# amin-abouee/apex-solver

Measured on AMD Instinct MI355X. Metric: ms per LM iter (Jacobian+Schur+solve), lower is better.
Workload: dtype f64; 1 GPU; final-13682 synthetic (13682 cameras / 4456117 landmarks / 28966251 observations); optimization_type=selfcal, camera_dof=9, schur_variant=sparse, s_tile_rows=856, s_tiles=8071, s_tiles_touched=4284, etree_levels=41, border_cameras=0, schur_form=4, variant_asked=Sparse, reason=, variant_choice=direct, parallelism=landmark-shard x1

## Files before the change

apex-solver_amd/csrc/chol_kernels.hip:

```cpp
#include <hip/hip_runtime.h>
#include <stdint.h>

#include "chol_kernels.h"
#include "device_reduce.hpp"
#include <algorithm>

namespace apex {

typedef double double4_t __attribute__((ext_vector_type(4)));

constexpr int NB = kNB;
constexpr int BS = 16;
constexpr int NBK = NB / BS;
constexpr int BP = 18;
constexpr int BSZ = BS * BP;
constexpr int NLB = NBK * (NBK + 1) / 2;

__device__ __forceinline__ int bidx(int bi, int bj) { return bi * (bi + 1) / 2 + bj; }

__device__ __forceinline__ double readlane_f64(double v, int src) {
    const int lo = __builtin_amdgcn_readlane(__double2loint(v), src);
    const int hi = __builtin_amdgcn_readlane(__double2hiint(v), src);
    return __hiloint2double(hi, lo);
}
// ... 183 lines not shown
                    Xm = __builtin_amdgcn_mfma_f64_16x16x4f64(-la, xb, Xm, 0, 0, 0);
                }
            }
            double* D = sA + bidx(kb, kb) * BSZ;
            double* Xd = sD + kb * BSZ;
#pragma unroll
            for (int r = 0; r < 4; ++r) {
                const int c = lk + 4 * r;
                D[lr * BP + c] = lr >= c ? Ls[r] : 0.0;
                Xd[c * BP + lr] = Xs[r];
            }
            if (isbad) *bad = 1;
            POTRF_STAMP();
        } else if (helper) {
            if (kb >= 1) {
                const int ks = kb - 1;
                for (int i = kb + 1 + hid; i < NBK; i += NH) {
                    double* Cb = sA + bidx(i, kb) * BSZ;
                    double4_t acc = blk_load_cd(Cb, lr, lk);
                    acc = blk_mma_nt(sA + bidx(i, ks) * BSZ, sA + bidx(kb, ks) * BSZ, acc, lr, lk, -1.0);
                    blk_store_cd(Cb, acc, lr, lk, 1.0);
                }
                const int m = NBK - 1 - kb;
                const int n_upd = m * (m + 1) / 2;
                for (int t = hid; t < n_upd; t += NH) {
                    int ii = 0;
                    while ((ii + 1) * (ii + 2) / 2 <= t) ++ii;
                    const int jj = t - ii * (ii + 1) / 2;
                    const int i = kb + 1 + ii, j = kb + 1 + jj;
                    double* Cb = sA + bidx(i, j) * BSZ;
                    double4_t acc = blk_load_cd(Cb, lr, lk);
                    acc = blk_mma_nt(sA + bidx(i, ks) * BSZ, sA + bidx(j, ks) * BSZ, acc, lr, lk, -1.0);
                    blk_store_cd(Cb, acc, lr, lk, 1.0);
                }
                const int r = ks;
                int nt = 0;
                for (int j = hid; j < r; j += NH, ++nt) {
                    double4_t acc = (double4_t){0.0, 0.0, 0.0, 0.0};
                    for (int k = j; k < r; ++k) {
                        const double* Y = (k == j) ? (sD + j * BSZ) : (sA + bidx(k, j) * BSZ);
                        acc = blk_mma_nn(sA + bidx(r, k) * BSZ, Y, acc, lr, lk);
                    }
                    T[nt] = acc;
                }
            }
        }
        __syncthreads();
        POTRF_STAMP();
        if (helper && kb >= 1) {
            const int r = kb - 1;
            int nt = 0;
            for (int j = hid; j < r; j += NH, ++nt) blk_store_cd(sA + bidx(r, j) * BSZ, T[nt], lr, lk, -1.0);
        }
        {
            const int m = NBK - 1 - kb;
            if (w == 0) {
                if (m > 0) {
                    double* N = sA + bidx(kb + 1, kb) * BSZ;
                    double4_t Lt = (double4_t){0.0, 0.0, 0.0, 0.0};
                    Lt = blk_mma_nt(sD + kb * BSZ, N, Lt, lr, lk, 1.0);
                    Dm = blk_load_cd_sym(sA + bidx(kb + 1, kb + 1) * BSZ, lr, lk);
#pragma unroll
                    for (int r = 0; r < 4; ++r) N[lr * BP + lk + 4 * r] = Lt[r];
#pragma unroll
                    for (int r = 0; r < 4; ++r) Dm = __builtin_amdgcn_mfma_f64_16x16x4f64(-Lt[r], Lt[r], Dm, 0, 0, 0);
                }
            } else if (helper) {
                const int t0 = m > 0 ? 1 : 0;
                for (int t = t0 + hid; t < m + kb; t += NH) {
                    if (t < m) {
                        double* P = sA + bidx(kb + 1 + t, kb) * BSZ;
                        double4_t acc = (double4_t){0.0, 0.0, 0.0, 0.0};
                        acc = blk_mma_nt(P, sD + kb * BSZ, acc, lr, lk, 1.0);
                        blk_store_cd(P, acc, lr, lk, 1.0);
                    } else {
                        const int k = t - m;
                        double* Bk = sA + bidx(kb, k) * BSZ;
                        blk_to_tile<COH>(Bk, A, rA, kb, k, lane, 64);
                        double4_t acc = (double4_t){0.0, 0.0, 0.0, 0.0};
                        acc = blk_mma_nn(sD + kb * BSZ, Bk, acc, lr, lk);
                        blk_store_cd(Bk, acc, lr, lk, 1.0);
                    }
                }
                if (hid == NH - 1) blk_to_tile<COH>(sA + bidx(kb, kb) * BSZ, A, rA, kb, kb, lane, 64);
            }
        }
        if (w == 0 || helper) {
            __builtin_amdgcn_fence(__ATOMIC_RELEASE, "workgroup");
            if (lane == 0) __hip_atomic_fetch_add(sync_cnt, 1, __ATOMIC_RELAXED, __HIP_MEMORY_SCOPE_WORKGROUP);
        }
        if (helper) {
            const int target = (kb + 1) * (NH + 1);
            while (__hip_atomic_load(sync_cnt, __ATOMIC_RELAXED, __HIP_MEMORY_SCOPE_WORKGROUP) < target) __builtin_amdgcn_s_sleep(0);
            __builtin_amdgcn_fence(__ATOMIC_ACQUIRE, "workgroup");
        }
        POTRF_STAMP();
    }
    __syncthreads();
    {
        const int r = NBK - 1;
        double4_t T[(NBK - 1 + NW - 1) / NW];
        int nt = 0;
        for (int j = w; j < r; j += NW, ++nt) {
            double4_t acc = (double4_t){0.0, 0.0, 0.0, 0.0};
            for (int k = j; k < r; ++k) {
                const double* Y = (k == j) ? (sD + j * BSZ) : (sA + bidx(k, j) * BSZ);
                acc = blk_mma_nn(sA + bidx(r, k) * BSZ, Y, acc, lr, lk);
            }
            T[nt] = acc;
        }
        __syncthreads();
        nt = 0;
        for (int j = w; j < r; j += NW, ++nt) blk_store_cd(sA + bidx(r, j) * BSZ, T[nt], lr, lk, -1.0);
        __syncthreads();
    }
#pragma unroll
    for (int bi = 0; bi < NBK; ++bi) {
        const int per_row = 8 * (bi + 1), cnt = 16 * per_row;
        for (int idx = tid; idx < cnt; idx += NT) {
            const int rr = idx / per_row, c2 = idx - rr * per_row;
            const int bj = c2 >> 3;
            const double* src = ((bj == bi) ? (sD + bi * BSZ) : (sA + bidx(bi, bj) * BSZ)) + rr * BP + 2 * (c2 & 7);
            double2 v; v.x = src[0]; v.y = src[1];
            tile_st2<COH>(Linv, rL, (16 * bi + rr) * NB + 2 * c2, v);
        }
    }
    if (tid == 0 && *bad) atomicCAS(fail, 0, K + 1);
    POTRF_STAMP();
}

template <int NW>
__global__ __launch_bounds__(64 * NW) void k_potrf_inv_mf(const PotrfTask* __restrict__ tasks, int* __restrict__ fail,
                                                          int* __restrict__ arrived) {
    if (arrived != nullptr && threadIdx.x == 0) __hip_atomic_fetch_add(arrived, 1, __ATOMIC_RELAXED, __HIP_MEMORY_SCOPE_AGENT);
    POTRF_STAMP();
    __shared__ double sA[NLB * BSZ];
    __shared__ double sD[NBK * BSZ];
    __shared__ int bad, sync_cnt;
    const PotrfTask pt = tasks[blockIdx.x];
    potrf_tile_mf<NW, false>(pt.A, pt.Linv, pt.K, fail, sA, sD, &bad, &sync_cnt);
}
#undef POTRF_STAMP

constexpr int KC = 16;
constexpr int STRIP = 48;
constexpr int NSTRIP = NB / STRIP;
constexpr int kGemmSmallMax = 56;

typedef double __attribute__((address_space(1)))* GlobalF64;
typedef const double __attribute__((address_space(1)))* GlobalCF64;
typedef double f64x2_t __attribute__((ext_vector_type(2)));
typedef const f64x2_t __attribute__((address_space(1)))* GlobalCF64x2;

template <bool TRI>
__global__ __launch_bounds__(256, 3) void k_tile_gemm_nt(const GemmTask* __restrict__ tasks, int n_units, double alpha, double beta) {
    constexpr int P4 = KC + 2;
    constexpr int IMG = (NB + STRIP) * P4;
    __shared__ double sm[IMG];
    const int per_xcd = (n_units + 7) >> 3;
    const int unit = (blockIdx.x & 7) * per_xcd + (blockIdx.x >> 3);
    if ((int)(blockIdx.x >> 3) >= per_xcd || unit >= n_units) return;
    GemmTask tg = tasks[unit / NSTRIP];
    const bool first = (reinterpret_cast<uintptr_t>(tg.C) & 1) != 0;
    tg.C = reinterpret_cast<double*>(reinterpret_cast<uintptr_t>(tg.C) & ~uintptr_t(7));
    const int strip = unit % NSTRIP;
    const int tid = threadIdx.x, lane = tid & 63, w = __builtin_amdgcn_readfirstlane(tid >> 6);
    const int lr = lane & 15, lk = lane >> 4;
    GlobalCF64 Ag = (GlobalCF64)tg.A + (size_t)strip * STRIP * NB;
    GlobalCF64 Bg = (GlobalCF64)tg.B;
    constexpr int NACC = TRI ? 9 : 7;
    int cb[3];
    if (TRI) { cb[0] = 16 * (8 - w); cb[1] = 16 * (1 + w); cb[2] = w == 3 ? 0 : -16; }
    else { cb[0] = 32 * w; cb[1] = 32 * w + 16; cb[2] = 128; }
    const bool extra = TRI ? (w == 3) : (w < 3);
    double4_t acc[NACC];
#pragma unroll
    for (int j = 0; j < NACC; ++j) acc[j] = (double4_t){0.0, 0.0, 0.0, 0.0};
    constexpr int C2 = KC / 2, NR = (NB + STRIP) * C2 / 256, RPR = 256 / C2;
    static_assert((NB + STRIP) * C2 % 256 == 0 && 256 % C2 == 0 && NR == 6 && RPR == 32, "staging loop assumes whole rounds");
    const int r0 = tid / C2, c2 = tid % C2;
    const unsigned offB = r0 * NB + 2 * c2, offA = (r0 + 16) * NB + 2 * c2;
    GlobalCF64 p4 = r0 < 16 ? Bg + (size_t)(r0 + 128) * NB + 2 * c2 : Ag + (size_t)(r0 - 16) * NB + 2 * c2;
    const int dst0 = r0 * P4 + 2 * c2;
    f64x2_t rg[NR];
    auto gload = [&](int k0) {
#pragma unroll
        for (int i = 0; i < 4; ++i) rg[i] = *reinterpret_cast<GlobalCF64x2>(Bg + (offB + (unsigned)(RPR * i * NB + k0)));
        rg[4] = *reinterpret_cast<GlobalCF64x2>(p4 + k0);
        rg[5] = *reinterpret_cast<GlobalCF64x2>(Ag + (offA + (unsigned)k0));
    };
    auto stage = [&](double* img) {
#pragma unroll
        for (int i = 0; i < NR; ++i) { img[dst0 + RPR * i * P4] = rg[i].x; img[dst0 + RPR * i * P4 + 1] = rg[i].y; }
    };
    auto compute = [&](const double* img, int k0) {
        const double* sB = img;
        const double* sA = img + NB * P4;
#pragma unroll
        for (int kk = 0; kk < KC; kk += 4) {
            if (TRI) {
                if (k0 > cb[0]) continue;
                double av[3], bv[3];
#pragma unroll
                for (int i = 0; i < 3; ++i) av[i] = sA[(16 * i + lr) * P4 + kk + lk];
#pragma unroll
                for (int j = 0; j < 3; ++j) bv[j] = sB[((cb[j] < 0 ? 0 : cb[j]) + lr) * P4 + kk + lk];
#pragma unroll
                for (int j = 0; j < 3; ++j) {
                    if (k0 > cb[j]) continue;
#pragma unroll
                    for (int i = 0; i < 3; ++i)
                        acc[3 * i + j] = __builtin_amdgcn_mfma_f64_16x16x4f64(av[i], bv[j], acc[3 * i + j], 0, 0, 0);
                }
            } else {
                double av[3], bv[2];
#pragma unroll
                for (int i = 0; i < 3; ++i) av[i] = sA[(16 * i + lr) * P4 + kk + lk];
#pragma unroll
                for (int j = 0; j < 2; ++j) bv[j] = sB[(cb[j] + lr) * P4 + kk + lk];
#pragma unroll
                for (int i = 0; i < 3; ++i)
#pragma unroll
                    for (int j = 0; j < 2; ++j)
                        acc[2 * i + j] = __builtin_amdgcn_mfma_f64_16x16x4f64(av[i], bv[j], acc[2 * i + j], 0, 0, 0);
                if (extra) {
                    const double ax = sA[(16 * w + lr) * P4 + kk + lk], bx = sB[(128 + lr) * P4 + kk + lk];
                    acc[6] = __builtin_amdgcn_mfma_f64_16x16x4f64(ax, bx, acc[6], 0, 0, 0);
                }
            }
        }
    };
    gload(0);
    for (int k0 = 0; k0 < NB; k0 += KC) {
        __syncthreads();
        stage(sm);
        __syncthreads();
        if (k0 + KC < NB) gload(k0 + KC);
        compute(sm, k0);
    }
    GlobalF64 C = (GlobalF64)tg.C + (size_t)strip * STRIP * NB;
    auto brow = [&](int n) { return TRI ? 16 * (n / 3) : (n < 6 ? 16 * (n / 2) : 16 * w); };
    auto bcol = [&](int n) { return TRI ? cb[n % 3] : (n < 6 ? cb[n % 2] : 128); };
    if (beta == 0.0 || first) {
        const double zero = first ? 0.0 : -0.0;
#pragma unroll
        for (int n = 0; n < NACC; ++n) {
            if (TRI ? (n % 3 == 2 && !extra) : (n == 6 && !extra)) continue;
#pragma unroll
            for (int r = 0; r < 4; ++r) C[(size_t)(brow(n) + lk + 4 * r) * NB + bcol(n) + lr] = alpha * acc[n][r] + zero;
        }
        return;
    }
    if (TRI) {
#pragma unroll
        for (int n = 0; n < NACC; ++n) {
            if (n % 3 == 2 && !extra) continue;
#pragma unroll
            for (int r = 0; r < 4; ++r) {
                GlobalF64 p = C + (size_t)(brow(n) + lk + 4 * r) * NB + bcol(n) + lr;
                *p = alpha * acc[n][r] + beta * *p;
            }
        }
        return;
    }
    double cv[3][4];
#pragma unroll
    for (int n = 0; n < 2; ++n)
#pragma unroll
        for (int r = 0; r < 4; ++r) cv[n][r] = C[(size_t)(brow(n) + lk + 4 * r) * NB + bcol(n) + lr];
#pragma unroll
    for (int n = 0; n < NACC; ++n) {
        if (n + 2 < NACC && (n + 2 < 6 || extra)) {
#pragma unroll
            for (int r = 0; r < 4; ++r) cv[(n + 2) % 3][r] = C[(size_t)(brow(n + 2) + lk + 4 * r) * NB + bcol(n + 2) + lr];
        }
        if (n == 6 && !extra) continue;
#pragma unroll
        for (int r = 0; r < 4; ++r)
            C[(size_t)(brow(n) + lk + 4 * r) * NB + bcol(n) + lr] = alpha * acc[n][r] + beta * cv[n % 3][r];
    }
}

constexpr int KS = 48;
constexpr int PS = KS + 2;

__global__ __launch_bounds__(192) void k_tile_gemm_nt_small(const GemmTask* __restrict__ tasks, int n_units, double alpha,
                                                              double beta) {
    __shared__ double sA[48 * PS];
    __shared__ double sB[48 * PS];
    const int unit = blockIdx.x;
    if (unit >= n_units) return;
    GemmTask tg = tasks[unit / 9];
    const bool first = (reinterpret_cast<uintptr_t>(tg.C) & 1) != 0;
    tg.C = reinterpret_cast<double*>(reinterpret_cast<uintptr_t>(tg.C) & ~uintptr_t(7));
    if (first) beta = 0.0;
    const int blk = unit % 9, bi = blk / 3, bj = blk % 3;
    GlobalCF64 Ag = (GlobalCF64)tg.A + (size_t)bi * 48 * NB;
    GlobalCF64 Bg = (GlobalCF64)tg.B + (size_t)bj * 48 * NB;
    GlobalF64 C = (GlobalF64)tg.C + (size_t)bi * 48 * NB + bj * 48;
    const int tid = threadIdx.x, lane = tid & 63, w = tid >> 6;
    const int lr = lane & 15, lk = lane >> 4;
    double4_t acc[3];
#pragma unroll
    for (int j = 0; j < 3; ++j) acc[j] = (double4_t){0.0, 0.0, 0.0, 0.0};
    constexpr int C2 = KS / 2, NR = 48 * C2 / 192;
    static_assert(48 * C2 % 192 == 0 && NB % KS == 0, "staging loops assume whole rounds");
    f64x2_t ra[NR], rb[NR];
    auto gload = [&](int k0) {
#pragma unroll
        for (int i = 0; i < NR; ++i) {
            const int idx = tid + 192 * i, row = idx / C2, c2 = idx % C2;
            ra[i] = *reinterpret_cast<GlobalCF64x2>(Ag + (size_t)row * NB + k0 + 2 * c2);
            rb[i] = *reinterpret_cast<GlobalCF64x2>(Bg + (size_t)row * NB + k0 + 2 * c2);
        }
    };
    double cv[3][4];
    if (beta != 0.0) {
#pragma unroll
        for (int j = 0; j < 3; ++j)
#pragma unroll
            for (int r = 0; r < 4; ++r) cv[j][r] = C[(size_t)(16 * w + lk + 4 * r) * NB + 16 * j + lr];
    }
    gload(0);
    for (int k0 = 0; k0 < NB; k0 += KS) {
        __syncthreads();
#pragma unroll
        for (int i = 0; i < NR; ++i) {
            const int idx = tid + 192 * i, row = idx / C2, c2 = idx % C2;
            sA[row * PS + 2 * c2] = ra[i].x; sA[row * PS + 2 * c2 + 1] = ra[i].y;
            sB[row * PS + 2 * c2] = rb[i].x; sB[row * PS + 2 * c2 + 1] = rb[i].y;
        }
        __syncthreads();
        if (k0 + KS < NB) gload(k0 + KS);
#pragma unroll
        for (int kk = 0; kk < KS; kk += 4) {
            const double a = sA[(16 * w + lr) * PS + kk + lk];
#pragma unroll
            for (int j = 0; j < 3; ++j) {
                const double b = sB[(16 * j + lr) * PS + kk + lk];
                acc[j] = __builtin_amdgcn_mfma_f64_16x16x4f64(a, b, acc[j], 0, 0, 0);
            }
        }
    }
#pragma unroll
    for (int j = 0; j < 3; ++j)
#pragma unroll
        for (int r = 0; r < 4; ++r) {
            const double v = alpha * acc[j][r];
            C[(size_t)(16 * w + lk + 4 * r) * NB + 16 * j + lr] = (beta != 0.0) ? v + beta * cv[j][r] : (first ? v + 0.0 : v);
        }
}

__global__ __launch_bounds__(576) void k_tile_gemm_nt_small_strip(const GemmTask* __restrict__ tasks, int n_units, double alpha,
                                                                    double beta) {
    __shared__ double sA[48 * PS];
    __shared__ double sB[NB * PS];
    const int unit = blockIdx.x;
    if (unit >= n_units) return;
    const GemmTask tg = tasks[unit / 3];
    const int bi = unit % 3;
    GlobalCF64 Ag = (GlobalCF64)tg.A + (size_t)bi * 48 * NB;
    GlobalCF64 Bg = (GlobalCF64)tg.B;
    GlobalF64 C = (GlobalF64)tg.C + (size_t)bi * 48 * NB;
    const int tid = threadIdx.x, lane = tid & 63, w = tid >> 6;
    const int lr = lane & 15, lk = lane >> 4;
    const int wr = w / 3, wc = w % 3;
    double4_t acc[3];
#pragma unroll
    for (int j = 0; j < 3; ++j) acc[j] = (double4_t){0.0, 0.0, 0.0, 0.0};
    constexpr int C2 = KS / 2, NRA = 48 * C2 / 576, NRB = NB * C2 / 576;
    static_assert(48 * C2 % 576 == 0 && NB * C2 % 576 == 0, "staging loops assume whole rounds");
    f64x2_t ra[NRA], rb[NRB];
    auto gload = [&](int k0) {
#pragma unroll
        for (int i = 0; i < NRA; ++i) {
            const int idx = tid + 576 * i, row = idx / C2, c2 = idx % C2;
            ra[i] = *reinterpret_cast<GlobalCF64x2>(Ag + (size_t)row * NB + k0 + 2 * c2);
        }
#pragma unroll
        for (int i = 0; i < NRB; ++i) {
            const int idx = tid + 576 * i, row = idx / C2, c2 = idx % C2;
            rb[i] = *reinterpret_cast<GlobalCF64x2>(Bg + (size_t)row * NB + k0 + 2 * c2);
        }
    };
    gload(0);
    for (int k0 = 0; k0 < NB; k0 += KS) {
        __syncthreads();
#pragma unroll
        for (int i = 0; i < NRA; ++i) {
            const int idx = tid + 576 * i, row = idx / C2, c2 = idx % C2;
            sA[row * PS + 2 * c2] = ra[i].x; sA[row * PS + 2 * c2 + 1] = ra[i].y;
        }
#pragma unroll
        for (int i = 0; i < NRB; ++i) {
            const int idx = tid + 576 * i, row = idx / C2, c2 = idx % C2;
            sB[row * PS + 2 * c2] = rb[i].x; sB[row * PS + 2 * c2 + 1] = rb[i].y;
        }
        __syncthreads();
        if (k0 + KS < NB) gload(k0 + KS);
#pragma unroll
        for (int kk = 0; kk < KS; kk += 4) {
            const double a = sA[(16 * wr + lr) * PS + kk + lk];
#pragma unroll
            for (int j = 0; j < 3; ++j) {
                const double b = sB[(48 * wc + 16 * j + lr) * PS + kk + lk];
                acc[j] = __builtin_amdgcn_mfma_f64_16x16x4f64(a, b, acc[j], 0, 0, 0);
            }
        }
    }
#pragma unroll
    for (int j = 0; j < 3; ++j)
#pragma unroll
        for (int r = 0; r < 4; ++r) {
            GlobalF64 dst = C + (size_t)(16 * wr + lk + 4 * r) * NB + 48 * wc + 16 * j + lr;
            const double v = alpha * acc[j][r];
            *dst = (beta != 0.0) ? v + beta * *dst : v;
        }
}

constexpr int HROWS = NB / 2;
constexpr int TP = NB + 1;

template <bool TRANS>
__device__ __forceinline__ void tile_gemv_lds(const double* __restrict__ M, const double* sv, double* sout, double* sT,
                                              double* spart, int tid) {
    double accT = 0.0;
    for (int h = 0; h < 2; ++h) {
        double2 reg[21];
#pragma unroll
        for (int i = 0; i < 21; ++i) {
            const int idx = tid + 256 * i;
            if (idx < HROWS * (NB / 2)) {
                const int row = idx / (NB / 2), c2 = idx - row * (NB / 2);
                reg[i] = *reinterpret_cast<const double2*>(M + (size_t)(HROWS * h + row) * NB + 2 * c2);
            }
        }
        __syncthreads();
#pragma unroll
        for (int i = 0; i < 21; ++i) {
            const int idx = tid + 256 * i;
            if (idx < HROWS * (NB / 2)) {
                const int row = idx / (NB / 2), c2 = idx - row * (NB / 2);
                sT[row * TP + 2 * c2] = reg[i].x; sT[row * TP + 2 * c2 + 1] = reg[i].y;
            }
        }
        __syncthreads();
        if (!TRANS) {
            if (tid < NB) {
                const int row = tid % HROWS, ch = tid / HROWS;
                double a = 0.0;
#pragma unroll 8
                for (int c = 0; c < HROWS; ++c) a += sT[row * TP + ch * HROWS + c] * sv[ch * HROWS + c];
                spart[ch * HROWS + row] = a;
            }
            __syncthreads();
            if (tid < HROWS) sout[HROWS * h + tid] = spart[tid] + spart[HROWS + tid];
        } else {
            if (tid < NB) {
#pragma unroll 8
                for (int r = 0; r < HROWS; ++r) accT += sT[r * TP + tid] * sv[HROWS * h + r];
            }
        }
    }
    if (TRANS && tid < NB) sout[tid] = accT;
    __syncthreads();
}

template <bool TRANS>
__global__ __launch_bounds__(256) void k_tri_step(const TriTask* __restrict__ tasks, int n_tasks, double* __restrict__ vwork,
                                                    double* __restrict__ vout) {
    __shared__ double sT[HROWS * TP];
    __shared__ double sv[NB], sy[NB], sz[NB], spart[NB];
    const int per_xcd = (n_tasks + 7) >> 3;
    const int unit = (blockIdx.x & 7) * per_xcd + (blockIdx.x >> 3);
    if ((int)(blockIdx.x >> 3) >= per_xcd || unit >= n_tasks) return;
    const TriTask t = tasks[unit];
    const int tid = threadIdx.x;
    if (tid < NB) sv[tid] = vwork[(size_t)t.k * NB + tid];
    __syncthreads();
    tile_gemv_lds<TRANS>(t.Mdiag, sv, sy, sT, spart, tid);
    if (t.other < 0) {
        if (tid < NB) vout[(size_t)t.k * NB + tid] = sy[tid];
        return;
    }
    tile_gemv_lds<TRANS>(t.Moff, sy, sz, sT, spart, tid);
    if (tid < NB) {
        if (!TRANS) unsafeAtomicAdd(&vwork[(size_t)t.other * NB + tid], -sz[tid]);
        else vwork[(size_t)t.other * NB + tid] -= sz[tid];
    }
}

__device__ __forceinline__ double flow_ld(const double* p) { return __hip_atomic_load(p, __ATOMIC_RELAXED, __HIP_MEMORY_SCOPE_AGENT); }
__device__ __forceinline__ void flow_st(double* p, double v) { __hip_atomic_store(p, v, __ATOMIC_RELAXED, __HIP_MEMORY_SCOPE_AGENT); }
constexpr int kFlowSpinLimit = 1 << 21;
__device__ __forceinline__ void flow_wait(const int* flag, int want, int tid, int* err) {
    if (tid == 0) {
        int spins = 0;
        while (__hip_atomic_load(flag, __ATOMIC_RELAXED, __HIP_MEMORY_SCOPE_AGENT) < want) {
            __builtin_amdgcn_s_sleep(1);
            if (++spins > kFlowSpinLimit) { atomicOr(err, 1); break; }
// ... 103 lines not shown
    }
    __syncthreads();
    spart[p][2 * j2] = a0; spart[p][2 * j2 + 1] = a1;
    __syncthreads();
    if (tid < NB) {
        double v = 0.0;
#pragma unroll
        for (int q = 0; q < kBwdParts; ++q) v += spart[q][tid];
        flow_st(t.src >= 0 ? part + (size_t)t.part * NB + tid : x + (size_t)t.dst * NB + tid, v);
    }
    flow_publish(t.src >= 0 ? cnt + t.dst : done + t.dst, tid);
}

template <int CTRL>
__device__ __forceinline__ double dpp_add(double v) {
    const int lo = __builtin_amdgcn_update_dpp(0, __double2loint(v), CTRL, 0xf, 0xf, true);
    const int hi = __builtin_amdgcn_update_dpp(0, __double2hiint(v), CTRL, 0xf, 0xf, true);
    return v + __hiloint2double(hi, lo);
}
__device__ __forceinline__ double row16_sum_lane15(double v) {
    v = dpp_add<0x111>(v);
    v = dpp_add<0x112>(v);
    v = dpp_add<0x114>(v);
    v = dpp_add<0x118>(v);
    return v;
}

constexpr int kFwdThreads = 576, kFwdRows = 4, kFwdCols = NB / 16;

__global__ __launch_bounds__(kFwdThreads) void k_tri_fwd_flow(const FlowTask* __restrict__ tasks, const double* __restrict__ b,
                                                             double* __restrict__ y, double* __restrict__ part,
                                                             int* __restrict__ cnt, int* __restrict__ done, int* __restrict__ err,
                                                             const double* __restrict__ fold_b, double* __restrict__ fold_out) {
    __shared__ double sx[NB];
    __shared__ double spart[4][NB];
    __shared__ double sinl[NB];
    const FlowTask t = tasks[blockIdx.x];
    const int tid = threadIdx.x, lane = tid & 63, w = tid >> 6;
    const int rg = lane >> 4, cl = lane & 15;
    const int row0 = 16 * w + kFwdRows * rg;
    const bool inl = t.src == -1 && t.src2 >= 0;
    double m[kFwdRows][kFwdCols], m2[kFwdRows][kFwdCols];
    {
        const double* __restrict__ M = t.mat + (size_t)row0 * NB + cl;
#pragma unroll
        for (int rr = 0; rr < kFwdRows; ++rr)
#pragma unroll
            for (int k = 0; k < kFwdCols; ++k) m[rr][k] = M[(size_t)rr * NB + 16 * k];
        const double* __restrict__ M2 = (inl ? t.mat2 : t.mat) + (size_t)row0 * NB + cl;
#pragma unroll
        for (int rr = 0; rr < kFwdRows; ++rr)
#pragma unroll
            for (int k = 0; k < kFwdCols; ++k) m2[rr][k] = inl ? M2[(size_t)rr * NB + 16 * k] : 0.0;
    }
    auto matvec = [&](const double (&mm)[kFwdRows][kFwdCols], double (&acc)[kFwdRows]) {
#pragma unroll
        for (int rr = 0; rr < kFwdRows; ++rr) acc[rr] = 0.0;
#pragma unroll
        for (int k = 0; k < kFwdCols; ++k) {
            const double xv = sx[cl + 16 * k];
#pragma unroll
            for (int rr = 0; rr < kFwdRows; ++rr) acc[rr] = fma(mm[rr][k], xv, acc[rr]);
        }
#pragma unroll
        for (int rr = 0; rr < kFwdRows; ++rr) acc[rr] = row16_sum_lane15(acc[rr]);
    };
    if (t.src >= 0) {
        flow_wait(done + t.src, 1, tid, err);
        if (tid < NB) sx[tid] = flow_ld(y + (size_t)t.src * NB + tid);
    } else {
        if (inl) {
            flow_wait2(cnt + t.dst, t.count - 1, done + t.src2, 1, tid, err);
            if (tid < NB) sx[tid] = flow_ld(y + (size_t)t.src2 * NB + tid);
            __syncthreads();
            double a2[kFwdRows];
            matvec(m2, a2);
            if (cl == 15) {
#pragma unroll
                for (int rr = 0; rr < kFwdRows; ++rr) sinl[row0 + rr] = a2[rr];
            }
            __syncthreads();
        } else {
            flow_wait(cnt + t.dst, t.count, tid, err);
        }
        const int g = tid / NB, c = tid - g * NB;
        const int s2 = inl ? t.slot2 : -1;
        double v = 0.0;
        {
            const double* __restrict__ pp = part + (size_t)t.part * NB + c;
            const double own = inl ? sinl[c] : 0.0;
            auto slot = [&](int q) { const double pv = flow_ld(pp + (size_t)q * NB); return q == s2 ? own : pv; };
            int q = g;
            for (; q + 12 < t.count; q += 16) {
                const double p0 = slot(q), p1 = slot(q + 4);
                const double p2 = slot(q + 8), p3 = slot(q + 12);
                v += (p0 + p1) + (p2 + p3);
            }
            for (; q < t.count; q += 4) v += slot(q);
        }
        spart[g][c] = v;
        __syncthreads();
        if (tid < NB) {
            const double* __restrict__ bsrc = t.src == -2 ? fold_b : b;
            const double rhs = bsrc ? bsrc[(size_t)t.dst * NB + tid] : 0.0;
            const double val = rhs - ((spart[0][tid] + spart[1][tid]) + (spart[2][tid] + spart[3][tid]));
            if (t.src == -2) fold_out[(size_t)t.dst * NB + tid] = val;
            else sx[tid] = val;
        }
        if (t.src == -2) return;
    }
    __syncthreads();
    double acc[kFwdRows];
    matvec(m, acc);
    if (cl == 15) {
        double* __restrict__ o = (t.src >= 0 ? part + (size_t)t.part * NB : y + (size_t)t.dst * NB) + row0;
#pragma unroll
        for (int rr = 0; rr < kFwdRows; ++rr) flow_st(o + rr, acc[rr]);
    }
    flow_publish(t.src >= 0 ? cnt + t.dst : done + t.dst, tid);
}

__device__ __forceinline__ void flow_wait_ge(const int* ver, int flag, int want, int tid, int* err) {
    if (flag >= 0) flow_wait(ver + flag, want, tid, err);
}
__device__ __forceinline__ void flow_wait_unit(const int* ver, const FactorUnit& u, int tid, int* err) {
    const int f0 = u.wait_flag[0], f1 = u.wait_flag[1], f2 = u.wait_flag[2], w0 = u.wait_val[0], w1 = u.wait_val[1], w2 = u.wait_val[2];
    if (tid < 64) {
        const int f = tid == 0 ? f0 : (tid == 1 ? f1 : (tid == 2 ? f2 : -1));
        const int want = tid == 0 ? w0 : (tid == 1 ? w1 : w2);
        int spins = 0;
        for (;;) {
            const bool ok = f < 0 || __hip_atomic_load(ver + f, __ATOMIC_RELAXED, __HIP_MEMORY_SCOPE_AGENT) >= want;
            if (__all(ok)) break;
            const bool dead = tid == 3 && __hip_atomic_load(err, __ATOMIC_RELAXED, __HIP_MEMORY_SCOPE_AGENT) != 0;
            if (__any(dead)) break;
            __builtin_amdgcn_s_sleep(1);
            if (++spins > kFlowSpinLimit) { if (tid == 0) atomicOr(err, 1); break; }
        }
    }
    __syncthreads();
}

constexpr int kFlowFactorThreadsC = 768;
constexpr int kFlowPK = NB + 2;
__device__ __forceinline__ void flow_update_unit(const FactorUnit& u, double* __restrict__ sA, double* __restrict__ sB,
                                                 int* __restrict__ ver, int* __restrict__ err, unsigned long long* __restrict__ trace) {
    const int tid = threadIdx.x, lane = tid & 63, w = tid >> 6;
    const int lr = lane & 15, lk = lane >> 4;
    const int wr = w / 3, wc = w % 3;
    const int bi = u.strip / 3, bj = u.strip % 3;
    const __amdgpu_buffer_rsrc_t rC = coh_rsrc(u.C), rA = coh_rsrc(u.A), rB = coh_rsrc(u.B);
    flow_wait_unit(ver, u, tid, err);
    if (trace && tid == 0) trace[1] = wall_clock64();
    const bool act = tid < 576;
    double cv[4] = {0.0, 0.0, 0.0, 0.0};
    if (act && !(u.kind & kFlowFirstWriter)) {
#pragma unroll
        for (int r = 0; r < 4; ++r) cv[r] = coh_ld1(rC, (48 * bi + 16 * wr + lk + 4 * r) * NB + 48 * bj + 16 * wc + lr);
    }
    constexpr int C2 = NB / 2, NR = 48 * C2 / 576;
    static_assert(48 * C2 % 576 == 0, "staging loops assume whole rounds");
    if (act) {
        double2 ra[NR], rb[NR];
#pragma unroll
        for (int i = 0; i < NR; ++i) {
            const int idx = tid + 576 * i, row = idx / C2, c2 = idx % C2;
            ra[i] = tile_ld2<true>(u.A, rA, (48 * bi + row) * NB + 2 * c2);
            rb[i] = tile_ld2<true>(u.B, rB, (48 * bj + row) * NB + 2 * c2);
        }
#pragma unroll
        for (int i = 0; i < NR; ++i) {
            const int idx = tid + 576 * i, row = idx / C2, c2 = idx % C2;
            sA[row * kFlowPK + 2 * c2] = ra[i].x; sA[row * kFlowPK + 2 * c2 + 1] = ra[i].y;
            sB[row * kFlowPK + 2 * c2] = rb[i].x; sB[row * kFlowPK + 2 * c2 + 1] = rb[i].y;
        }
    }
    __syncthreads();
    if (act) {
        double4_t acc = (double4_t){0.0, 0.0, 0.0, 0.0};
        const double* pa = sA + (16 * wr + lr) * kFlowPK + lk;
        const double* pb = sB + (16 * wc + lr) * kFlowPK + lk;
#pragma unroll
        for (int kk = 0; kk < NB; kk += 4) acc = __builtin_amdgcn_mfma_f64_16x16x4f64(pa[kk], pb[kk], acc, 0, 0, 0);
#pragma unroll
        for (int r = 0; r < 4; ++r)
            coh_st1(rC, (48 * bi + 16 * wr + lk + 4 * r) * NB + 48 * bj + 16 * wc + lr, -1.0 * acc[r] + 1.0 * cv[r]);
    }
    flow_publish(ver + u.pub, tid);
}

__device__ __forceinline__ void flow_solve_unit(const FactorUnit& u, double* __restrict__ sA, double* __restrict__ sB,
                                                int* __restrict__ ver, int* __restrict__ err, unsigned long long* __restrict__ trace) {
    const int tid = threadIdx.x, lane = tid & 63, w = tid >> 6;
    const int lr = lane & 15, lk = lane >> 4;
    const int row0 = 16 * u.strip;
    const __amdgpu_buffer_rsrc_t rC = coh_rsrc(u.C), rB = coh_rsrc(u.B);
    constexpr int C2 = KS / 2, NCH = NB / KS, NRB = NB * C2 / 576;
    static_assert(NB * C2 % 576 == 0 && 16 * C2 <= 576, "staging loops assume whole rounds");
    flow_wait_unit(ver, u, tid, err);
    if (trace && tid == 0) trace[1] = wall_clock64();
    const bool act = tid < 576;
    double2 ra[NCH], rb[NCH][NRB];
#pragma unroll
    for (int c = 0; c < NCH; ++c)
        if (tid < 16 * C2) ra[c] = tile_ld2<true>(u.C, rC, (row0 + tid / C2) * NB + KS * c + 2 * (tid % C2));
    if (act) {
#pragma unroll
        for (int c = 0; c < NCH; ++c)
#pragma unroll
            for (int i = 0; i < NRB; ++i) {
                const int idx = tid + 576 * i, row = idx / C2, c2 = idx % C2;
                rb[c][i] = tile_ld2<true>(u.B, rB, row * NB + KS * c + 2 * c2);
            }
    }
    double4_t acc = (double4_t){0.0, 0.0, 0.0, 0.0};
#pragma unroll
    for (int c = 0; c < NCH; ++c) {
        __syncthreads();
        if (tid < 16 * C2) { const int row = tid / C2, c2 = tid % C2; sA[row * PS + 2 * c2] = ra[c].x; sA[row * PS + 2 * c2 + 1] = ra[c].y; }
        if (act) {
#pragma unroll
            for (int i = 0; i < NRB; ++i) {
                const int idx = tid + 576 * i, row = idx / C2, c2 = idx % C2;
                sB[row * PS + 2 * c2] = rb[c][i].x; sB[row * PS + 2 * c2 + 1] = rb[c][i].y;
            }
        }
        __syncthreads();
        if (act) {
#pragma unroll
            for (int kk = 0; kk < KS; kk += 4)
                acc = __builtin_amdgcn_mfma_f64_16x16x4f64(sA[lr * PS + kk + lk], sB[(16 * w + lr) * PS + kk + lk], acc, 0, 0, 0);
        }
    }
    if (act) {
#pragma unroll
        for (int r = 0; r < 4; ++r) coh_st1(rC, (row0 + lk + 4 * r) * NB + 16 * w + lr, acc[r]);
    }
    flow_publish(ver + u.pub, tid);
}


__device__ __forceinline__ void flow_update_tile_unit(const FactorUnit& u, double* __restrict__ sA, double* __restrict__ sB,
                                                      int* __restrict__ ver, int* __restrict__ err, unsigned long long* __restrict__ trace) {
    const int tid = threadIdx.x, lane = tid & 63, w = tid >> 6;
    const int lr = lane & 15, lk = lane >> 4;
    const __amdgpu_buffer_rsrc_t rC = coh_rsrc(u.C), rA = coh_rsrc(u.A), rB = coh_rsrc(u.B);
    flow_wait_unit(ver, u, tid, err);
    if (trace && tid == 0) trace[1] = wall_clock64();
    constexpr int NBW = 7;
    const int nb = w < 9 ? 7 : 6, b0 = w < 9 ? 7 * w : 63 + 6 * (w - 9);
    constexpr int C2 = KS / 2, NCH = NB / KS;
    constexpr int NLD = (NB * C2 + kFlowFactorThreadsC - 1) / kFlowFactorThreadsC;
    double2 ra[NLD], rb[NLD];
    auto load_chunk = [&](int c) {
#pragma unroll
        for (int i = 0; i < NLD; ++i) {
            const int idx = tid + kFlowFactorThreadsC * i, row = min(idx / C2, NB - 1), c2 = idx % C2;
            ra[i] = tile_ld2<true>(u.A, rA, row * NB + KS * c + 2 * c2);
            rb[i] = tile_ld2<true>(u.B, rB, row * NB + KS * c + 2 * c2);
        }
    };
    load_chunk(0);
    double4_t acc[NBW];
#pragma unroll
    for (int q = 0; q < NBW; ++q) acc[q] = (double4_t){0.0, 0.0, 0.0, 0.0};
    double cv[NBW][4];
#pragma unroll
    for (int c = 0; c < NCH; ++c) {
        __syncthreads();
#pragma unroll
        for (int i = 0; i < NLD; ++i) {
            const int idx = tid + kFlowFactorThreadsC * i, row = idx / C2, c2 = idx % C2;
            if (idx < NB * C2) {
                sA[row * PS + 2 * c2] = ra[i].x; sA[row * PS + 2 * c2 + 1] = ra[i].y;
                sB[row * PS + 2 * c2] = rb[i].x; sB[row * PS + 2 * c2 + 1] = rb[i].y;
            }
        }
        if (c + 1 < NCH) {
            load_chunk(c + 1);
        } else {
            const bool first = (u.kind & kFlowFirstWriter) != 0;
#pragma unroll
            for (int q = 0; q < NBW; ++q) {
                const int b = min(b0 + q, 80), br = b / 9, bc = b - 9 * br;
#pragma unroll
                for (int r = 0; r < 4; ++r) cv[q][r] = first ? 0.0 : coh_ld1(rC, (16 * br + lk + 4 * r) * NB + 16 * bc + lr);
            }
        }
        __syncthreads();
#pragma unroll
        for (int q = 0; q < NBW; ++q) {
            if (q < nb) {
                const int b = b0 + q, br = b / 9, bc = b - 9 * br;
                const double* pa = sA + (16 * br + lr) * PS + lk;
                const double* pb = sB + (16 * bc + lr) * PS + lk;
#pragma unroll
                for (int kk = 0; kk < KS; kk += 4) acc[q] = __builtin_amdgcn_mfma_f64_16x16x4f64(pa[kk], pb[kk], acc[q], 0, 0, 0);
            }
        }
    }
#pragma unroll
    for (int q = 0; q < NBW; ++q) {
        if (q < nb) {
            const int b = b0 + q, br = b / 9, bc = b - 9 * br;
#pragma unroll
            for (int r = 0; r < 4; ++r) coh_st1(rC, (16 * br + lk + 4 * r) * NB + 16 * bc + lr, -1.0 * acc[q][r] + 1.0 * cv[q][r]);
        }
    }
    __builtin_amdgcn_s_waitcnt(0);
    __syncthreads();
    if (tid == 0) __hip_atomic_fetch_add(ver + u.pub, kFlowUnitsPerTile, __ATOMIC_RELAXED, __HIP_MEMORY_SCOPE_AGENT);
}

constexpr int kFlowFactorThreads = 768;
__global__ __launch_bounds__(kFlowFactorThreads) void k_factor_flow(const FactorUnit* __restrict__ units, int* __restrict__ ver,
                                                                     int* __restrict__ fail, int* __restrict__ err,
                                                                     unsigned long long* __restrict__ trace) {
    __shared__ double smem[(NLB + NBK) * BSZ];
    __shared__ int bad, sync_cnt;
    static_assert((16 + NB) * PS <= (NLB + NBK) * BSZ && 2 * 48 * kFlowPK <= (NLB + NBK) * BSZ && 2 * NB * PS <= (NLB + NBK) * BSZ, "the products' staging areas fit in the potrf's");
    static_assert(kFlowFactorThreadsC == kFlowFactorThreads, "one constant");
    const FactorUnit u = units[blockIdx.x];
    const int tid = threadIdx.x;
    if (trace) {
        trace += 3 * (size_t)blockIdx.x;
        if (tid == 0) trace[0] = wall_clock64();
    }
    const int kind = u.kind & 15;
    if (kind == 0) {
        flow_wait_unit(ver, u, tid, err);
        if (trace && tid == 0) trace[1] = wall_clock64();
        potrf_tile_mf<kFlowFactorThreads / 64, true>(u.C, const_cast<double*>(u.A), u.strip, fail, smem, smem + NLB * BSZ, &bad, &sync_cnt);
        __builtin_amdgcn_s_waitcnt(0);
        __syncthreads();
        if (tid == 0) __hip_atomic_fetch_add(ver + u.pub, kFlowUnitsPerTile, __ATOMIC_RELAXED, __HIP_MEMORY_SCOPE_AGENT);
    } else if (kind == 1) {
        flow_solve_unit(u, smem, smem + 16 * PS, ver, err, trace);
    } else if (kind == 3) {
        flow_update_tile_unit(u, smem, smem + NB * PS, ver, err, trace);
    } else {
        flow_update_unit(u, smem, smem + 48 * kFlowPK, ver, err, trace);
    }
    if (trace && tid == 0) trace[2] = wall_clock64();
}

template <int CTRL, int ROW_MASK>
__device__ __forceinline__ double sym_dpp_add(double x) {
    const int lo = __builtin_amdgcn_update_dpp(0, __double2loint(x), CTRL, ROW_MASK, 0xF, true);
    const int hi = __builtin_amdgcn_update_dpp(0, __double2hiint(x), CTRL, ROW_MASK, 0xF, true);
    return x + __hiloint2double(hi, lo);
}
__device__ __forceinline__ double sym_wave_sum(double x) {
    x = sym_dpp_add<0x118, 0xF>(x);
    x = sym_dpp_add<0x114, 0xF>(x);
    x = sym_dpp_add<0x112, 0xF>(x);
    x = sym_dpp_add<0x111, 0xF>(x);
    x = sym_dpp_add<0x142, 0xA>(x);
    x = sym_dpp_add<0x143, 0xC>(x);
    return x;
}
__global__ __launch_bounds__(256) void k_sym_tile_products(const SymTile* __restrict__ list,
                                                             const double* __restrict__ tiles,
                                                             const double* __restrict__ x, double* __restrict__ part) {
    constexpr int RW = NB / 4;
    constexpr int RB = 6;
    __shared__ double sxI[NB], su[NB], sv[4][NB];
    const SymTile st = list[blockIdx.x];
    const double* __restrict__ M = tiles + (size_t)st.slot * (NB * NB);
    const int tid = threadIdx.x, lane = tid & 63, w = tid >> 6;
    const bool diag = (st.I == st.J);
    if (tid < NB) sxI[tid] = x[(size_t)st.I * NB + tid];
    const bool ext = lane < 8;
    const int c0 = 2 * lane, c1 = 128 + 2 * lane;
    const double2 xj = *reinterpret_cast<const double2*>(x + (size_t)st.J * NB + c0);
    const double2 xje = ext ? *reinterpret_cast<const double2*>(x + (size_t)st.J * NB + c1) : make_double2(0.0, 0.0);
    double v0 = 0.0, v1 = 0.0, ve0 = 0.0, ve1 = 0.0;
    __syncthreads();
    for (int rb = 0; rb < RW; rb += RB) {
        double2 m[RB], me[RB];
#pragma unroll
        for (int k = 0; k < RB; ++k) {
            const double* row = M + (size_t)(RW * w + rb + k) * NB;
            m[k] = *reinterpret_cast<const double2*>(row + c0);
            me[k] = ext ? *reinterpret_cast<const double2*>(row + c1) : make_double2(0.0, 0.0);
        }
#pragma unroll
        for (int k = 0; k < RB; ++k) {
            const int r = RW * w + rb + k;
            double a0 = m[k].x, a1 = m[k].y, b0 = me[k].x, b1 = me[k].y;
            if (diag) {
                if (c0 > r) a0 = 0.0;
                if (c0 + 1 > r) a1 = 0.0;
                if (c1 > r) b0 = 0.0;
                if (c1 + 1 > r) b1 = 0.0;
            }
            const double pr = fma(a0, xj.x, fma(a1, xj.y, fma(b0, xje.x, b1 * xje.y)));
            const double tot = sym_wave_sum(pr);
            if (lane == 63) su[r] = tot;
            if (diag) {
                if (c0 == r) a0 = 0.0;
                if (c0 + 1 == r) a1 = 0.0;
                if (c1 == r) b0 = 0.0;
                if (c1 + 1 == r) b1 = 0.0;
            }
            const double xi = sxI[r];
            v0 = fma(a0, xi, v0); v1 = fma(a1, xi, v1); ve0 = fma(b0, xi, ve0); ve1 = fma(b1, xi, ve1);
        }
    }
    sv[w][c0] = v0; sv[w][c0 + 1] = v1;
    if (ext) { sv[w][c1] = ve0; sv[w][c1 + 1] = ve1; }
    __syncthreads();
    double* pu = part + (size_t)st.slot * (2 * NB);
    if (tid < NB) {
        pu[tid] = su[tid];
        pu[NB + tid] = (sv[0][tid] + sv[1][tid]) + (sv[2][tid] + sv[3][tid]);
    }
}

__global__ __launch_bounds__(256) void k_sym_tile_gather(const int* __restrict__ row_ptr,
                                                           const SymEntry* __restrict__ entries,
                                                           const double* __restrict__ part,
                                                           const double* __restrict__ p, double* __restrict__ y,
                                                           double* __restrict__ row_dot) {
    __shared__ double sc[4];
    const int I = blockIdx.x, tid = threadIdx.x;
    double acc = 0.0;
    if (tid < NB) {
        for (int e = row_ptr[I]; e < row_ptr[I + 1]; ++e) {
            const SymEntry en = entries[e];
            const double* pu = part + (size_t)en.slot * (2 * NB);
            if (en.kind == 0) acc += pu[tid];
            else if (en.kind == 1) acc += pu[NB + tid];
            else acc += pu[tid] + pu[NB + tid];
        }
        y[(size_t)I * NB + tid] = acc;
    }
    double d = (tid < NB) ? acc * p[(size_t)I * NB + tid] : 0.0;
    d = wave_sum(d);
    if ((tid & 63) == 0) sc[tid >> 6] = d;
    __syncthreads();
    if (tid == 0) row_dot[I] = (sc[0] + sc[1]) + (sc[2] + sc[3]);
}

__global__ __launch_bounds__(256) void k_pcg_step1(int n, int nt, const double* __restrict__ scal,
                                                     const double* __restrict__ row_dot, const double* __restrict__ p,
                                                     const double* __restrict__ ap, const double* __restrict__ pre,
                                                     double* __restrict__ x, double* __restrict__ r,
                                                     double* __restrict__ blk_part, double* __restrict__ out_pap) {
    __shared__ double sc[4];
    __shared__ double s_alpha;
    const int tid = threadIdx.x;
    double pap = 0.0;
    for (int i = tid; i < nt; i += 256) pap += row_dot[i];
    pap = wave_sum(pap);
    if ((tid & 63) == 0) sc[tid >> 6] = pap;
    __syncthreads();
    if (tid == 0) {
// ... 360 lines not shown
```

Baseline: 12.23 ms.

## Exploit symmetry in diagonal SYRK-style tile updates to compute only lower blocks

When a tile GEMM has A equal to B (a diagonal Schur-complement update), the kernels now compute and store only the lower-triangular 16x16 blocks. The strip GEMM gets a dedicated path whose per-strip wave assignment is a constexpr table checked at compile time. The small GEMM skips upper blocks, and the flow factor units load B once and reuse it. This roughly halves MFMA work and global loads on diagonal tiles, but leaves the upper triangle unwritten, so it relies on downstream code reading only the lower part. The dealt work across waves is also less balanced.

Measured after the change: 39.46 ms. 223% more time.

```diff
diff --git a/apex-solver_amd/csrc/chol_kernels.hip b/apex-solver_amd/csrc/chol_kernels.hip
--- a/apex-solver_amd/csrc/chol_kernels.hip
+++ b/apex-solver_amd/csrc/chol_kernels.hip
@@ -359,6 +359,124 @@
 typedef double f64x2_t __attribute__((ext_vector_type(2)));
 typedef const f64x2_t __attribute__((address_space(1)))* GlobalCF64x2;
 
+
+struct SymDeal { int col[2], rows[2], extra; };
+constexpr SymDeal kSymDeal[NSTRIP][4] = {
+    {{{0, 0}, {3, 0}, -1}, {{0, 2}, {4, 4}, -1}, {{1, 0}, {2, 0}, -1}, {{1, 0}, {4, 0}, -1}},
+    {{{0, 5}, {7, 4}, -1}, {{1, 4}, {7, 2}, -1}, {{2, 4}, {7, 4}, -1}, {{3, 0}, {7, 0}, -1}},
+    {{{0, 1}, {7, 7}, -1}, {{2, 3}, {7, 7}, -1}, {{4, 5}, {7, 7}, -1}, {{6, 7}, {7, 6}, 8}},
+};
+constexpr bool sym_deal_is_exact() {
+    for (int s = 0; s < NSTRIP; ++s) {
+        int seen[3][NBK] = {}, needed = 0, worst = 0;
+        for (int w = 0; w < 4; ++w) {
+            const SymDeal& d = kSymDeal[s][w];
+            int mine = 0;
+            for (int j = 0; j < 2; ++j)
+                for (int i = 0; i < 3; ++i)
+                    if (d.rows[j] >> i & 1) { ++seen[i][d.col[j]]; ++mine; }
+            if (d.extra >= 0) { ++seen[2][d.extra]; ++mine; }
+            worst = mine > worst ? mine : worst;
+        }
+        for (int i = 0; i < 3; ++i)
+            for (int c = 0; c < NBK; ++c) {
+                const int want = c <= 3 * s + i ? 1 : 0;
+                if (seen[i][c] != want) return false;
+                needed += want;
+            }
+        if (worst > (needed + 3) / 4 + 1) return false;
+    }
+    return true;
+}
+static_assert(sym_deal_is_exact(), "the deal of the diagonal strips");
+
+__device__ __forceinline__ void gemm_strip_sym(const double* Bt, double* Ct, int strip, bool first, double alpha, double beta,
+                                               double* sm) {
+    constexpr int P4 = KC + 2, C2 = KC / 2, RPR = 256 / C2;
+    const int tid = threadIdx.x, lane = tid & 63, w = __builtin_amdgcn_readfirstlane(tid >> 6);
+    const int lr = lane & 15, lk = lane >> 4;
+    GlobalCF64 Bg = (GlobalCF64)Bt;
+    const SymDeal deal = kSymDeal[strip][w];
+    const int cb[2] = {16 * deal.col[0], 16 * deal.col[1]}, rows[2] = {deal.rows[0], deal.rows[1]};
+    const bool extra = deal.extra >= 0;
+    const int cx = extra ? 16 * deal.extra : 0;
+    auto active = [&](int n) { return n < 6 ? (rows[n / 3] >> (n % 3) & 1) != 0 : extra; };
+    double4_t acc[7];
+#pragma unroll
+    for (int j = 0; j < 7; ++j) acc[j] = (double4_t){0.0, 0.0, 0.0, 0.0};
+    const int r0 = tid / C2, c2 = tid % C2, n_rows = STRIP * (strip + 1);
+    const unsigned offB = r0 * NB + 2 * c2;
+    const int dst0 = r0 * P4 + 2 * c2;
+    constexpr int NR = (NB + RPR - 1) / RPR;
+    f64x2_t rg[NR];
+    auto gload = [&](int k0) {
+#pragma unroll
+        for (int i = 0; i < NR; ++i)
+            if (r0 + RPR * i < n_rows) rg[i] = *reinterpret_cast<GlobalCF64x2>(Bg + (offB + (unsigned)(RPR * i * NB + k0)));
+    };
+    auto stage = [&](double* img) {
+#pragma unroll
+        for (int i = 0; i < NR; ++i)
+            if (r0 + RPR * i < n_rows) { img[dst0 + RPR * i * P4] = rg[i].x; img[dst0 + RPR * i * P4 + 1] = rg[i].y; }
+    };
+    const double* sA = sm + STRIP * strip * P4;
+    gload(0);
+    for (int k0 = 0; k0 < NB; k0 += KC) {
+        __syncthreads();
+        stage(sm);
+        __syncthreads();
+        if (k0 + KC < NB) gload(k0 + KC);
+#pragma unroll
+        for (int kk = 0; kk < KC; kk += 4) {
+            double av[3], bv[2];
+#pragma unroll
+            for (int i = 0; i < 3; ++i) av[i] = sA[(16 * i + lr) * P4 + kk + lk];
+#pragma unroll
+            for (int j = 0; j < 2; ++j) bv[j] = sm[(cb[j] + lr) * P4 + kk + lk];
+#pragma unroll
+            for (int j = 0; j < 2; ++j)
+#pragma unroll
+                for (int i = 0; i < 3; ++i)
+                    if (active(3 * j + i)) acc[3 * j + i] = __builtin_amdgcn_mfma_f64_16x16x4f64(av[i], bv[j], acc[3 * j + i], 0, 0, 0);
+            if (extra) {
+                const double bx = sm[(cx + lr) * P4 + kk + lk];
+                acc[6] = __builtin_amdgcn_mfma_f64_16x16x4f64(av[2], bx, acc[6], 0, 0, 0);
+            }
+        }
+    }
+    GlobalF64 C = (GlobalF64)Ct + (size_t)strip * STRIP * NB;
+    auto brow = [&](int n) { return n < 6 ? 16 * (n % 3) : 32; };
+    auto bcol = [&](int n) { return n < 6 ? cb[n / 3] : cx; };
+    if (beta == 0.0 || first) {
+        const double zero = first ? 0.0 : -0.0;
+#pragma unroll
+        for (int n = 0; n < 7; ++n) {
+            if (!active(n)) continue;
+#pragma unroll
+            for (int r = 0; r < 4; ++r) C[(size_t)(brow(n) + lk + 4 * r) * NB + bcol(n) + lr] = alpha * acc[n][r] + zero;
+        }
+        return;
+    }
+    double cv[3][4];
+#pragma unroll
+    for (int n = 0; n < 2; ++n) {
+        if (!active(n)) continue;
+#pragma unroll
+        for (int r = 0; r < 4; ++r) cv[n][r] = C[(size_t)(brow(n) + lk + 4 * r) * NB + bcol(n) + lr];
+    }
+#pragma unroll
+    for (int n = 0; n < 7; ++n) {
+        if (n + 2 < 7 && active(n + 2)) {
+#pragma unroll
+            for (int r = 0; r < 4; ++r) cv[(n + 2) % 3][r] = C[(size_t)(brow(n + 2) + lk + 4 * r) * NB + bcol(n + 2) + lr];
+        }
+        if (!active(n)) continue;
+#pragma unroll
+        for (int r = 0; r < 4; ++r)
+            C[(size_t)(brow(n) + lk + 4 * r) * NB + bcol(n) + lr] = alpha * acc[n][r] + beta * cv[n % 3][r];
+    }
+}
+
 template <bool TRI>
 __global__ __launch_bounds__(256, 3) void k_tile_gemm_nt(const GemmTask* __restrict__ tasks, int n_units, double alpha, double beta) {
     constexpr int P4 = KC + 2;
@@ -371,6 +489,9 @@
     const bool first = (reinterpret_cast<uintptr_t>(tg.C) & 1) != 0;
     tg.C = reinterpret_cast<double*>(reinterpret_cast<uintptr_t>(tg.C) & ~uintptr_t(7));
     const int strip = unit % NSTRIP;
+    if constexpr (!TRI) {
+        if (tg.A == tg.B) { gemm_strip_sym(tg.B, tg.C, strip, first, alpha, beta, sm); return; }
+    }
     const int tid = threadIdx.x, lane = tid & 63, w = __builtin_amdgcn_readfirstlane(tid >> 6);
     const int lr = lane & 15, lk = lane >> 4;
     GlobalCF64 Ag = (GlobalCF64)tg.A + (size_t)strip * STRIP * NB;
@@ -502,11 +623,14 @@
     tg.C = reinterpret_cast<double*>(reinterpret_cast<uintptr_t>(tg.C) & ~uintptr_t(7));
     if (first) beta = 0.0;
     const int blk = unit % 9, bi = blk / 3, bj = blk % 3;
+    const bool sym = tg.A == tg.B;
+    if (sym && bj > bi) return;
     GlobalCF64 Ag = (GlobalCF64)tg.A + (size_t)bi * 48 * NB;
     GlobalCF64 Bg = (GlobalCF64)tg.B + (size_t)bj * 48 * NB;
     GlobalF64 C = (GlobalF64)tg.C + (size_t)bi * 48 * NB + bj * 48;
-    const int tid = threadIdx.x, lane = tid & 63, w = tid >> 6;
+    const int tid = threadIdx.x, lane = tid & 63, w = __builtin_amdgcn_readfirstlane(tid >> 6);
     const int lr = lane & 15, lk = lane >> 4;
+    const int nj = (sym && bi == bj) ? w + 1 : 3;
     double4_t acc[3];
 #pragma unroll
     for (int j = 0; j < 3; ++j) acc[j] = (double4_t){0.0, 0.0, 0.0, 0.0};
@@ -526,7 +650,7 @@
 #pragma unroll
         for (int j = 0; j < 3; ++j)
 #pragma unroll
-            for (int r = 0; r < 4; ++r) cv[j][r] = C[(size_t)(16 * w + lk + 4 * r) * NB + 16 * j + lr];
+            for (int r = 0; r < 4; ++r) if (j < nj) cv[j][r] = C[(size_t)(16 * w + lk + 4 * r) * NB + 16 * j + lr];
     }
     gload(0);
     for (int k0 = 0; k0 < NB; k0 += KS) {
@@ -544,6 +668,7 @@
             const double a = sA[(16 * w + lr) * PS + kk + lk];
 #pragma unroll
             for (int j = 0; j < 3; ++j) {
+                if (j >= nj) continue;
                 const double b = sB[(16 * j + lr) * PS + kk + lk];
                 acc[j] = __builtin_amdgcn_mfma_f64_16x16x4f64(a, b, acc[j], 0, 0, 0);
             }
@@ -553,6 +678,7 @@
     for (int j = 0; j < 3; ++j)
 #pragma unroll
         for (int r = 0; r < 4; ++r) {
+            if (j >= nj) continue;
             const double v = alpha * acc[j][r];
             C[(size_t)(16 * w + lk + 4 * r) * NB + 16 * j + lr] = (beta != 0.0) ? v + beta * cv[j][r] : (first ? v + 0.0 : v);
         }
@@ -962,9 +1088,11 @@
     const __amdgpu_buffer_rsrc_t rC = coh_rsrc(u.C), rA = coh_rsrc(u.A), rB = coh_rsrc(u.B);
     flow_wait_unit(ver, u, tid, err);
     if (trace && tid == 0) trace[1] = wall_clock64();
-    const bool act = tid < 576;
+    const bool sym = u.A == u.B;
+    const bool act = tid < 576 && !(sym && bj > bi);
+    const bool mine = act && !(sym && wc > wr);
     double cv[4] = {0.0, 0.0, 0.0, 0.0};
-    if (act && !(u.kind & kFlowFirstWriter)) {
+    if (mine && !(u.kind & kFlowFirstWriter)) {
 #pragma unroll
         for (int r = 0; r < 4; ++r) cv[r] = coh_ld1(rC, (48 * bi + 16 * wr + lk + 4 * r) * NB + 48 * bj + 16 * wc + lr);
     }
@@ -986,7 +1114,7 @@
         }
     }
     __syncthreads();
-    if (act) {
+    if (mine) {
         double4_t acc = (double4_t){0.0, 0.0, 0.0, 0.0};
         const double* pa = sA + (16 * wr + lr) * kFlowPK + lk;
         const double* pb = sB + (16 * wc + lr) * kFlowPK + lk;
@@ -1058,7 +1186,13 @@
     flow_wait_unit(ver, u, tid, err);
     if (trace && tid == 0) trace[1] = wall_clock64();
     constexpr int NBW = 7;
-    const int nb = w < 9 ? 7 : 6, b0 = w < 9 ? 7 * w : 63 + 6 * (w - 9);
+    const bool sym = u.A == u.B;
+    const int nb = sym ? (w < 9 ? 4 : 3) : (w < 9 ? 7 : 6);
+    const int b0 = sym ? (w < 9 ? 4 * w : 36 + 3 * (w - 9)) : (w < 9 ? 7 * w : 63 + 6 * (w - 9));
+    auto block_of = [&](int b, int& br, int& bc) {
+        if (sym) { br = 0; while ((br + 1) * (br + 2) / 2 <= b) ++br; bc = b - br * (br + 1) / 2; }
+        else { br = b / 9; bc = b - 9 * br; }
+    };
     constexpr int C2 = KS / 2, NCH = NB / KS;
     constexpr int NLD = (NB * C2 + kFlowFactorThreadsC - 1) / kFlowFactorThreadsC;
     double2 ra[NLD], rb[NLD];
@@ -1067,9 +1201,10 @@
         for (int i = 0; i < NLD; ++i) {
             const int idx = tid + kFlowFactorThreadsC * i, row = min(idx / C2, NB - 1), c2 = idx % C2;
             ra[i] = tile_ld2<true>(u.A, rA, row * NB + KS * c + 2 * c2);
-            rb[i] = tile_ld2<true>(u.B, rB, row * NB + KS * c + 2 * c2);
+            if (!sym) rb[i] = tile_ld2<true>(u.B, rB, row * NB + KS * c + 2 * c2);
         }
     };
+    const double* sBr = sym ? sA : sB;
     load_chunk(0);
     double4_t acc[NBW];
 #pragma unroll
@@ -1083,7 +1218,7 @@
             const int idx = tid + kFlowFactorThreadsC * i, row = idx / C2, c2 = idx % C2;
             if (idx < NB * C2) {
                 sA[row * PS + 2 * c2] = ra[i].x; sA[row * PS + 2 * c2 + 1] = ra[i].y;
-                sB[row * PS + 2 * c2] = rb[i].x; sB[row * PS + 2 * c2 + 1] = rb[i].y;
+                if (!sym) { sB[row * PS + 2 * c2] = rb[i].x; sB[row * PS + 2 * c2 + 1] = rb[i].y; }
             }
         }
         if (c + 1 < NCH) {
@@ -1092,7 +1227,9 @@
             const bool first = (u.kind & kFlowFirstWriter) != 0;
 #pragma unroll
             for (int q = 0; q < NBW; ++q) {
-                const int b = min(b0 + q, 80), br = b / 9, bc = b - 9 * br;
+                if (q >= nb) continue;
+                int br, bc;
+                block_of(b0 + q, br, bc);
 #pragma unroll
                 for (int r = 0; r < 4; ++r) cv[q][r] = first ? 0.0 : coh_ld1(rC, (16 * br + lk + 4 * r) * NB + 16 * bc + lr);
             }
@@ -1101,9 +1238,10 @@
 #pragma unroll
         for (int q = 0; q < NBW; ++q) {
             if (q < nb) {
-                const int b = b0 + q, br = b / 9, bc = b - 9 * br;
+                int br, bc;
+                block_of(b0 + q, br, bc);
                 const double* pa = sA + (16 * br + lr) * PS + lk;
-                const double* pb = sB + (16 * bc + lr) * PS + lk;
+                const double* pb = sBr + (16 * bc + lr) * PS + lk;
 #pragma unroll
                 for (int kk = 0; kk < KS; kk += 4) acc[q] = __builtin_amdgcn_mfma_f64_16x16x4f64(pa[kk], pb[kk], acc[q], 0, 0, 0);
             }
@@ -1112,7 +1250,8 @@
 #pragma unroll
     for (int q = 0; q < NBW; ++q) {
         if (q < nb) {
-            const int b = b0 + q, br = b / 9, bc = b - 9 * br;
+            int br, bc;
+            block_of(b0 + q, br, bc);
 #pragma unroll
             for (int r = 0; r < 4; ++r) coh_st1(rC, (16 * br + lk + 4 * r) * NB + 16 * bc + lr, -1.0 * acc[q][r] + 1.0 * cv[q][r]);
         }
```
